# jenndrei/BayHunter

Hardware: AMD Instinct MI355X
Metric: forward-model+logL evals/sec (batched 10-layer models) (higher is better)
Workload: dtype f64

## Files before the change

bayhunter_amd/csrc/swd_fa.h:

```cpp
#pragma once

namespace fa {
constexpr double SIGN_FLOOR = 1.0e-12;

__device__ __forceinline__ void sqrt_rsqrt(double x, double &s, double &rs)
{
    const double y = __builtin_amdgcn_rsq(x);
    double g = x * y, h = 0.5 * y;
    double r = __builtin_fma(-h, g, 0.5);
    g = __builtin_fma(g, r, g);
    h = __builtin_fma(h, r, h);
    r = __builtin_fma(-h, g, 0.5);
    g = __builtin_fma(g, r, g);
    h = __builtin_fma(h, r, h);
    s = g;
    rs = h + h;
}
__device__ __forceinline__ double rcp(double x)
{
    double r = __builtin_amdgcn_rcp(x);
    r = __builtin_fma(r, __builtin_fma(-x, r, 1.0), r);
    return __builtin_fma(r, __builtin_fma(-x, r, 1.0), r);
}
__device__ __forceinline__ double rcp1(double x)
{
    const double r = __builtin_amdgcn_rcp(x);
    return __builtin_fma(r, __builtin_fma(-x, r, 1.0), r);
}

__device__ __forceinline__ void sincos(double x, double &sn, double &cs)
{
    const double n = __builtin_rint(x * 6.36619772367581382433e-01);
    double r = __builtin_fma(-n, 1.57079632673412561417e+00, x);
    r = __builtin_fma(-n, 6.07710050650619224932e-11, r);
    const double z = r * r, z2 = z * z, z4 = z2 * z2;
    const double s01 = __builtin_fma(z, 8.33333333332248946124e-03, -1.66666666666666324348e-01);
    const double s23 = __builtin_fma(z, 2.75573137070700676789e-06, -1.98412698298579493134e-04);
    const double s45 = __builtin_fma(z, 1.58969099521155010221e-10, -2.50507602534068634195e-08);
    const double ps = __builtin_fma(z4, s45, __builtin_fma(z2, s23, s01));
    const double s = __builtin_fma(r * z, ps, r);
    const double c01 = __builtin_fma(z, -1.38888888888741095749e-03, 4.16666666666666019037e-02);
    const double c23 = __builtin_fma(z, -2.75573143513906633035e-07, 2.48015872894767294178e-05);
    const double c45 = __builtin_fma(z, -1.13596475577881948265e-11, 2.08757232129817482790e-09);
    const double pc = __builtin_fma(z4, c45, __builtin_fma(z2, c23, c01));
    const double c = __builtin_fma(z2, pc, __builtin_fma(z, -0.5, 1.0));
    const int q = (int)n & 3;
    const double ss = (q & 1) ? c : s, cc = (q & 1) ? s : c;
    sn = (q & 2) ? -ss : ss;
    cs = ((q + 1) & 2) ? -cc : cc;
}
__device__ __forceinline__ double expneg(double x)
{
    const double t = -x;
    const double n = __builtin_rint(t * 1.44269504088896338700e+00);
    double r = __builtin_fma(-n, 6.93147180369123816490e-01, t);
    r = __builtin_fma(-n, 1.90821492927058770002e-10, r);
    const double r2 = r * r, r4 = r2 * r2, r8 = r4 * r4;
    const double p01 = __builtin_fma(r, 1.66666666666666666667e-01, 0.5);
    const double p23 = __builtin_fma(r, 8.33333333333333333333e-03, 4.16666666666666666667e-02);
    const double p45 = __builtin_fma(r, 1.98412698412698412698e-04, 1.38888888888888888889e-03);
    const double p67 = __builtin_fma(r, 2.75573192239858906526e-06, 2.48015873015873015873e-05);
    const double p89 = __builtin_fma(r, 2.50521083854417187751e-08, 2.75573192239858906526e-07);
    const double p03 = __builtin_fma(r2, p23, p01), p47 = __builtin_fma(r2, p67, p45);
    const double p8a = __builtin_fma(r2, 2.08767569878680989792e-09, p89);
    const double p = __builtin_fma(r8, p8a, __builtin_fma(r4, p47, p03));
    const double e = __builtin_fma(r2, p, r) + 1.0;
    return e * __longlong_as_double((long long)((unsigned long long)((long long)n + 1023ll) << 52));
}

__device__ __forceinline__ void wave(double k, double xk, double d, double &cs, double &w, double &x, double &em)
{
    const double dk = k - xk;
    const double r2 = (k + xk) * fabs(dk);
    const bool zero = !(r2 > 1.0e-290);
    double r, rr;
    sqrt_rsqrt(zero ? 1.0 : r2, r, rr);
    r = zero ? 0.0 : r;
    const double p = r * d;
    double sn;
    if (dk < 0.0) {
        sincos(fmin(p, 9.0e4), sn, cs);
        x = -(r * sn);
        em = 1.0;
    } else {
        em = expneg(fmin(p, 700.0));
        const double hf = 0.5 * (em * em);
        cs = 0.5 + hf;
        sn = 0.5 - hf;
        x = r * sn;
    }
    w = zero ? d : sn * rr;
    if (!(p < 9.0e4)) cs = __builtin_nan("");
}

__device__ __forceinline__ void layer_products(double wvno, double xka, double xkb, double dpth, LayerTerms &o)
{
    double cosp, w, x, ep, cosq, y, z, eq;
    wave(wvno, xka, dpth, cosp, w, x, ep);
    wave(wvno, xkb, dpth, cosq, y, z, eq);
    o.a0 = ep * eq;
    o.cpcq = cosp * cosq;
    o.cpy = cosp * y;
    o.cpz = cosp * z;
    o.cqw = cosq * w;
    o.cqx = cosq * x;
    o.xy = x * y;
    o.xz = x * z;
    o.wy = w * y;
    o.wz = w * z;
    o.w = w;
    o.cosp = cosp;
}

__device__ __forceinline__ void ca19(Ca19 &o, double wvno2, double gam, double gammk, double rho, double irho, const LayerTerms &v)
{
#pragma clang fp contract(fast)
    const double gamm1 = gam - 1.0;
    const double twgm1 = gam + gamm1;
    const double gmgmk = gam * gammk;
    const double gmgm1 = gam * gamm1;
    const double gm1sq = gamm1 * gamm1;
    const double rho2 = rho * rho, irho2 = irho * irho;
    const double a0pq = v.a0 - v.cpcq;
    const double ca11 = v.cpcq - 2.0 * gmgm1 * a0pq - gmgmk * v.xz - wvno2 * gm1sq * v.wy;
    const double ca12 = (wvno2 * v.cpy - v.cqx) * irho;
    const double ca13 = -(twgm1 * a0pq + gammk * v.xz + wvno2 * gamm1 * v.wy) * irho;
    const double ca14 = (v.cpz - wvno2 * v.cqw) * irho;
    const double ca15 = -(2.0 * wvno2 * a0pq + v.xz + wvno2 * wvno2 * v.wy) * irho2;
    const double ca21 = (gmgmk * v.cpz - gm1sq * v.cqw) * rho;
    const double ca23 = gammk * v.cpz - gamm1 * v.cqw;
    const double ca41 = (gm1sq * v.cpy - gmgmk * v.cqx) * rho;
    const double ca43 = gamm1 * v.cpy - gammk * v.cqx;
    const double ca51 = -(2.0 * gmgmk * gm1sq * a0pq + gmgmk * gmgmk * v.xz + gm1sq * gm1sq * v.wy) * rho2;
    const double ca53 = -(gammk * gamm1 * twgm1 * a0pq + gam * gammk * gammk * v.xz + gamm1 * gm1sq * v.wy) * rho;
    const double t = -2.0 * wvno2;
    o.c[0] = ca11; o.c[1] = ca12; o.c[2] = ca13; o.c[3] = ca14; o.c[4] = ca15;
    o.c[5] = ca21; o.c[6] = ca23; o.c[7] = -v.wz; o.c[8] = v.cpcq;
    o.c[9] = ca41; o.c[10] = -v.xy; o.c[11] = ca43;
    o.c[12] = ca51; o.c[13] = ca53;
    o.c[14] = t * ca53;
    o.c[15] = t * ca43;
    o.c[16] = v.a0 + 2.0 * (v.cpcq - ca11);
    o.c[17] = t * ca23;
    o.c[18] = t * ca13;
}

__device__ __forceinline__ void rayleigh_halfspace(double e[5], double wvno, double wvno2, double xka, double xkb, double gammk, double rho1)
{
#pragma clang fp contract(fast)
    const double ra2 = (wvno + xka) * fabs(wvno - xka), rb2 = (wvno + xkb) * fabs(wvno - xkb);
    double ra, rb, t;
    sqrt_rsqrt(ra2 > 1.0e-290 ? ra2 : 1.0, ra, t);
    sqrt_rsqrt(rb2 > 1.0e-290 ? rb2 : 1.0, rb, t);
    ra = ra2 > 1.0e-290 ? ra : 0.0;
    rb = rb2 > 1.0e-290 ? rb : 0.0;
    const double gam = gammk * wvno2;
    const double gamm1 = gam - 1.0;
    const double rarb = ra * rb;
    e[0] = rho1 * rho1 * (gamm1 * gamm1 - gam * gammk * rarb);
    e[1] = -rho1 * ra;
    e[2] = rho1 * (gamm1 - gammk * rarb);
    e[3] = rho1 * rb;
    e[4] = wvno2 - rarb;
}

__device__ __forceinline__ void normalize5(double v0, double v1, double v2, double v3, double v4, double e[5])
{
    double t1 = fmax(fmax(fmax(fabs(v0), fabs(v1)), fmax(fabs(v2), fabs(v3))), fabs(v4));
    if (t1 < 1.0e-40) t1 = 1.0;
    const double r = rcp1(t1);
    e[0] = v0 * r;
    e[1] = v1 * r;
    e[2] = v2 * r;
    e[3] = v3 * r;
    e[4] = v4 * r;
}

__device__ __forceinline__ void love_step(double &e1, double &e2, double cosq, double yx, double zx)
{
    const double e10 = __builtin_fma(e2, zx, e1 * cosq);
    const double e20 = __builtin_fma(e1, yx, e2 * cosq);
    double xnor = fmax(fabs(e10), fabs(e20));
    if (xnor < 1.0e-40) xnor = 1.0;
    const double r = rcp1(xnor);
    e1 = e10 * r;
    e2 = e20 * r;
}
__device__ __forceinline__ void love_terms(double wvno, double xkb, double dm, double &cosq, double &y, double &z, double &q)
{
    double em;
    const double dk = wvno - xkb;
    const double r2 = (wvno + xkb) * fabs(dk);
    const bool zero = !(r2 > 1.0e-290);
    double rb, rr;
    sqrt_rsqrt(zero ? 1.0 : r2, rb, rr);
    rb = zero ? 0.0 : rb;
    q = dm * rb;
    double sn;
    if (dk < 0.0) {
        sincos(fmin(q, 9.0e4), sn, cosq);
        z = -(rb * sn);
    } else {
        em = expneg(fmin(q, 700.0));
        const double hf = 0.5 * (em * em);
        cosq = 0.5 + hf;
        sn = 0.5 - hf;
        z = rb * sn;
    }
    y = zero ? dm : sn * rr;
    if (!(q < 9.0e4)) cosq = __builtin_nan("");
}

__device__ __forceinline__ void apply5(const double e[5], const double *c, double ee[5])
{
    const double ca11 = c[0], ca12 = c[1], ca13 = c[2], ca14 = c[3], ca15 = c[4];
    const double ca21 = c[5], ca23 = c[6], ca24 = c[7], ca22 = c[8];
    const double ca41 = c[9], ca42 = c[10], ca43 = c[11], ca51 = c[12], ca53 = c[13];
    const double ca31 = c[14], ca32 = c[15], ca33 = c[16], ca34 = c[17], ca35 = c[18];
    ee[0] = __builtin_fma(e[4], ca51, __builtin_fma(e[2], ca31, e[0] * ca11)) + __builtin_fma(e[3], ca41, e[1] * ca21);
    ee[1] = __builtin_fma(e[4], ca41, __builtin_fma(e[2], ca32, e[0] * ca12)) + __builtin_fma(e[3], ca42, e[1] * ca22);
    ee[2] = __builtin_fma(e[4], ca53, __builtin_fma(e[2], ca33, e[0] * ca13)) + __builtin_fma(e[3], ca43, e[1] * ca23);
    ee[3] = __builtin_fma(e[4], ca21, __builtin_fma(e[2], ca34, e[0] * ca14)) + __builtin_fma(e[3], ca22, e[1] * ca24);
    ee[4] = __builtin_fma(e[4], ca11, __builtin_fma(e[2], ca35, e[0] * ca15)) + __builtin_fma(e[3], ca12, e[1] * ca14);
}

template <class MD>
__device__ __forceinline__ double rayleigh_secular(double wvno, double omga, const MD &md, int mmax, int llw, int mtop)
{
    const double omega = omga < 1.0e-4 ? 1.0e-4 : omga;
    const double wvno2 = wvno * wvno;
    const double iom = rcp(omega);
    double e[5];
    {
        const double bh = md.Bv(mmax - 1);
        const double t = bh * iom;
        rayleigh_halfspace(e, wvno, wvno2, omega * rcp(md.A(mmax - 1)), omega * rcp(bh), 2.0 * t * t, md.R(mmax - 1));
    }
    for (int m = mtop - 2; m >= 0; --m) {
        if (m <= mmax - 2 && m >= llw - 1) {
            const double am = md.A(m), bm = md.Bv(m), rho1 = md.R(m), dpth = md.D(m);
            const double t = bm * iom;
            const double gammk = 2.0 * t * t;
            LayerTerms v;
            layer_products(wvno, omega * rcp(am), omega * rcp(bm), dpth, v);
            Ca19 c;
            ca19(c, wvno2, gammk * wvno2, gammk, rho1, rcp(rho1), v);
            double ee[5];
            apply5(e, c.c, ee);
            normalize5(ee[0], ee[1], ee[2], ee[3], ee[4], e);
        }
    }
    double result = e[0];
    if (llw != 1) {
        LayerTerms v;
        layer_products(wvno, omega * rcp(md.A(0)), wvno + 1.0, md.D(0), v);
        result = v.cosp * e[0] - md.R(0) * v.w * e[1];
    }
    return result;
}

template <class MD>
__device__ __forceinline__ double love_secular(double wvno, double omega, const MD &md, int mmax, int llw, int mtop, int *nv = nullptr)
{
    double e1, e2;
    LoveCount lc;
    {
        const double ib = rcp(md.Bv(mmax - 1));
        const double xkb = omega * ib;
        const double r2 = (wvno + xkb) * fabs(wvno - xkb);
        double rb, t_;
        sqrt_rsqrt(r2 > 1.0e-290 ? r2 : 1.0, rb, t_);
        rb = r2 > 1.0e-290 ? rb : 0.0;
        e1 = md.R(mmax - 1) * rb;
        e2 = ib * ib;
        lc.reset(wvno > xkb);
    }
    for (int m = mtop - 2; m >= 0; --m) {
        if (m <= mmax - 2 && m >= llw - 1) {
            const double beta1 = md.Bv(m), rho1 = md.R(m);
            const double ib = rcp(beta1);
            const double xkb = omega * ib;
            double cosq, y, z, q;
            love_terms(wvno, xkb, md.D(m), cosq, y, z, q);
            const double fl = (wvno < xkb) ? love_zero_floor(q) : 0.0;
            const double e2o = e2;
            love_step(e1, e2, cosq, y * (ib * ib * rcp(rho1)), z * (rho1 * beta1 * beta1));
            lc.layer(fl, e2o, e2);
        }
    }
    if (nv != nullptr) *nv = lc.packed(e1, e2);
    return e1;
}
}
```

bayhunter_amd/csrc/swd_lean.hip:

```cpp
#include "../../include/bh_engine_debug.h"
#include "bh_device.h"
#include "bh_tuning.h"
#include <algorithm>
#define BH_HD __device__ __forceinline__
#define BH_TAB static __device__ const
#include "bh_libm.h"

namespace {
#include "swd_common.h"

struct LeanModel {
    const double *p;
    int S, LS;
    __device__ __forceinline__ double D(int m) const { return p[m * S]; }
    __device__ __forceinline__ double A(int m) const { return p[LS + m * S]; }
    __device__ __forceinline__ double Bv(int m) const { return p[2 * LS + m * S]; }
    __device__ __forceinline__ double R(int m) const { return p[3 * LS + m * S]; }
    __device__ __forceinline__ double IA(int m) const { return p[4 * LS + m * S]; }
    __device__ __forceinline__ double IB(int m) const { return p[5 * LS + m * S]; }
    __device__ __forceinline__ double IR(int m) const { return p[6 * LS + m * S]; }
};

__device__ __forceinline__ double lean_rayleigh(double wvno, double omega, double iom, const LeanModel &md, int mmax, int mtop)
{
    const double wvno2 = wvno * wvno;
    double e[5];
    {
        const double t = md.Bv(mmax - 1) * iom;
        fa::rayleigh_halfspace(e, wvno, wvno2, omega * md.IA(mmax - 1), omega * md.IB(mmax - 1), 2.0 * t * t, md.R(mmax - 1));
    }
    for (int m = mtop - 2; m >= 0; --m) {
        if (m <= mmax - 2) {
            const double t = md.Bv(m) * iom;
            const double gammk = 2.0 * t * t;
            LayerTerms v;
            fa::layer_products(wvno, omega * md.IA(m), omega * md.IB(m), md.D(m), v);
            Ca19 c;
            fa::ca19(c, wvno2, gammk * wvno2, gammk, md.R(m), md.IR(m), v);
            double ee[5];
            fa::apply5(e, c.c, ee);
            if ((m & 1) == 0) {
                fa::normalize5(ee[0], ee[1], ee[2], ee[3], ee[4], e);
            } else {
#pragma unroll
                for (int i = 0; i < 5; ++i) e[i] = ee[i];
            }
        }
    }
    return e[0];
}
__device__ __forceinline__ double lean_love(double wvno, double omega, const LeanModel &md, int mmax, int mtop)
{
    double e1, e2;
    {
        const double ib = md.IB(mmax - 1);
        const double xkb = omega * ib;
        const double r2 = (wvno + xkb) * fabs(wvno - xkb);
        double rb, t_;
        fa::sqrt_rsqrt(r2 > 1.0e-290 ? r2 : 1.0, rb, t_);
        rb = r2 > 1.0e-290 ? rb : 0.0;
        e1 = md.R(mmax - 1) * rb;
        e2 = ib * ib;
    }
    for (int m = mtop - 2; m >= 0; --m) {
        if (m <= mmax - 2) {
            const double ib = md.IB(m), bm = md.Bv(m), rho1 = md.R(m);
            double cosq, y, z, q;
            fa::love_terms(wvno, omega * ib, md.D(m), cosq, y, z, q);
            fa::love_step(e1, e2, cosq, y * (ib * ib * md.IR(m)), z * (rho1 * bm * bm));
        }
    }
    return e1;
}

enum : int {
    PH_START = 0,
    PH_SCAN = 1,
    PH_REF1 = 2,
    PH_REFC = 3,
    PH_PROBE_STEP = 4,
    PH_PROBE_ACC = 5,
    PH_SPECIAL = 6,
    PH_PROBE_START = 7,
    PH_SPECIAL_B = 8,
    PH_SPECIAL_C = 9
};

__device__ __forceinline__ bool sign_neg(double x) { return __double_as_longlong(x) < 0; }
__device__ __forceinline__ void lean_wave_sync()
{
    __builtin_amdgcn_fence(__ATOMIC_RELEASE, "wavefront");
    __builtin_amdgcn_wave_barrier();
    __builtin_amdgcn_fence(__ATOMIC_ACQUIRE, "wavefront");
}

#ifndef BH_LEAN_CLUSTER_W
#define BH_LEAN_CLUSTER_W 4.0e-7
#endif
#ifndef BH_LEAN_RIDE_TOL
#define BH_LEAN_RIDE_TOL 4.0e-7
#endif
#ifndef BH_LEAN_CLUSTER_BIG
#define BH_LEAN_CLUSTER_BIG 8
#endif
#ifndef BH_LEAN_CLUSTER
#define BH_LEAN_CLUSTER 2
#endif
constexpr int LEAN_WPB = 4;

template <int J, bool CNT>
__global__ __launch_bounds__(BH_WAVE * LEAN_WPB) void swd_lean_kernel(SwdMultiArgs A, int wave_lds, int flip)
{
    if (A.started != nullptr && threadIdx.x == 0) atomicAdd(A.started, 1u);
    const int lane = threadIdx.x & (BH_WAVE - 1);
    const int wave = __builtin_amdgcn_readfirstlane((int)(threadIdx.x / BH_WAVE));
    int wid = (int)blockIdx.x * LEAN_WPB + wave, ty = (int)blockIdx.y;
    if (A.wg_n1 > 0) {
        const long long n1 = A.wg_n1, N = (long long)A.wg_n0 + n1;
        if (wid >= (int)N) return;
        const int l0 = (int)(((long long)wid * n1) / N), l1 = (int)((((long long)wid + 1) * n1) / N);
        ty = (l1 > l0) ? 1 : 0;
        wid = (l1 > l0) ? l0 : wid - l0;
        if ((flip & 256) && ty == 1) {
            if (flip & 2048) {
                const int x = (wid >> 1) & 7, q = ((wid >> 4) << 1) | (wid & 1), qr = A.wg_n1 / 8 - 1 - q;
                wid = ((qr >> 1) << 4) + 2 * x + (qr & 1);
            } else {
                wid = A.wg_n1 - 1 - wid;
            }
        }
    }
    const SwdTarget T = A.t[ty];
    constexpr int MPW = BH_WAVE / J;
    if (wid * MPW >= A.B) return;
    const int g = lane / J, r = lane & (J - 1), lbase = lane & ~(J - 1);
    const int sidx = wid * MPW + g;
    const bool valid = sidx < A.B;
    const int32_t *perm = T.perm != nullptr ? T.perm : A.perm;
    const int ib = valid ? (perm ? perm[sidx] : sidx) : 0;
    const int Lmax = A.Lmax, K = T.K, ifunc = T.iwave;
    extern __shared__ __align__(16) unsigned char smem_lean[];
    double *omg = reinterpret_cast<double *>(smem_lean + (size_t)wave * wave_lds);
    double *mdl = omg + ((K + 1) & ~1);
    const int LS = Lmax * MPW;
    constexpr double dc = (double)0.005f, onea = (double)1.5f, twopi = 2.0 * 3.141592653589793, guard_rel = 3.0e-6;
    for (int k = lane; k < K; k += BH_WAVE) omg[k] = twopi / T.periods[k];
    for (int idx = lane; idx < LS; idx += BH_WAVE) {
        const int l = idx / MPW, mg = idx - l * MPW;
        const int sb = wid * MPW + mg;
        const int b = sb < A.B ? (perm ? perm[sb] : sb) : 0;
        float fd = 0.f, fa_ = 1.f, fb = 1.f, fr = 1.f;
        if (sb < A.B && l < A.nlay[b]) {
            const ptrdiff_t o = (ptrdiff_t)b * T.sb + (ptrdiff_t)l * T.sl;
            fd = (float)T.h[o];
            fa_ = (float)T.vp[o];
            fb = (float)T.vs[o];
            fr = (float)T.rho[o];
        }
        mdl[idx] = (double)fd;
        mdl[LS + idx] = (double)fa_;
        mdl[2 * LS + idx] = (double)fb;
        mdl[3 * LS + idx] = (double)fr;
        mdl[4 * LS + idx] = fa::rcp((double)fa_);
        mdl[5 * LS + idx] = fa::rcp((double)fb);
        mdl[6 * LS + idx] = fa::rcp((double)fr);
    }
    int mmax = valid ? A.nlay[ib] : 2;
    mmax = mmax < 1 ? 1 : (mmax > Lmax ? Lmax : mmax);
    int mtop = mmax;
    for (int off = 32; off > 0; off >>= 1) mtop = max(mtop, __shfl_xor(mtop, off));
    mtop = __builtin_amdgcn_readfirstlane(mtop);
    lean_wave_sync();
    LeanModel md;
    md.p = mdl + g;
    md.S = MPW;
    md.LS = LS;

    float betmx = -1.e20f, betmn = 1.e20f;
    int jmn = 0, jsol = 1;
    bool sane = true;
    for (int i = 0; i < mmax; ++i) {
        const float bi = (float)md.Bv(i), ai = (float)md.A(i), di = (float)md.D(i), ri = (float)md.R(i);
        sane = sane && (ai > 0.0f) && (ai <= 100.0f) && (bi >= 0.0f) && (bi <= 100.0f) && (ri > 0.0f) && (ri < 1.0e6f) &&
               (i == mmax - 1 || (di >= 0.0f && di < 1.0e7f));
        if (bi > 0.01f && bi < betmn) {
            betmn = bi;
            jmn = i;
            jsol = 1;
        } else if (bi <= 0.01f && ai < betmn) {
            betmn = ai;
            jmn = i;
            jsol = 0;
        }
        if (bi > betmx) betmx = bi;
    }
    float cc1 = (jsol == 0) ? betmn : gtsolh_f32((float)md.A(jmn), (float)md.Bv(jmn));
    cc1 = 0.95f * cc1;
    cc1 = 0.90f * cc1;
    const double cm = (double)cc1, betmxd = (double)betmx;
    const double vh0 = md.Bv(mmax - 1), vh1 = (ifunc == 2) ? md.A(mmax - 1) : betmxd, vsafe = fmin(vh0, vh1);
    auto special_in_cell = [&](double lo_, double hi_) -> double {
        double sp = 0.0;
        int n = 0;
        if (lo_ < betmxd && betmxd < hi_) sp = betmxd, ++n;
        if (vh0 != betmxd && lo_ < vh0 && vh0 < hi_) sp = vh0, ++n;
        if (vh1 != betmxd && vh1 != vh0 && lo_ < vh1 && vh1 < hi_) sp = vh1, ++n;
        return n > 1 ? -1.0 : sp;
    };
    double *vel = T.vel + (size_t)ib * T.ldv;
    const bool writer = valid && r == 0;
    bool active = valid && K > 0 && sane, guard = false;
#define LEAN_GUARD(n) do { guard = true; if (CNT) greason = (n); } while (0)
    int greason = 0;
    int errflag = 0;
    if (valid && !sane) {
        errflag = 1;
        if (writer)
            for (int i = 0; i < K; ++i) vel[i] = 0.0;
    }
    if (active && md.Bv(0) <= 0.0) {
        LEAN_GUARD(1);
        active = false;
    }
    int k = 0, ph = PH_START, idir = +1, ifirst = 1, nref = 0;
    double c1 = cm, clow = cm, del1 = 0.0, ck = 0.0, omega = 1.0, iom = 1.0;
    bool s1stneg = false;
    double cp = 0.0, delp = 0.0;
    bool havep = false;
    double lo = 0.0, hi = 0.0, flo = 0.0, fhi = 0.0, p3 = 0.0, fp3 = 0.0, c3 = 0.0, wprev = 0.0;
    bool have3 = false;
    double cell_lo = 0.0, cell_hi = 0.0, pb = 0.0, delb = 0.0;
    bool pp_neg = false;
    int sp_nb = 0;
    bool flo_neg = false, chk = false;
    unsigned evals = 0;
    if (active) {
        omega = omg[0];
        iom = fa::rcp(omega);
    }
    constexpr unsigned long long maskJ = (J >= 64) ? ~0ull : ((1ull << J) - 1ull);
    constexpr int NC = (J >= 32) ? BH_LEAN_CLUSTER_BIG : ((J >= 8) ? BH_LEAN_CLUSTER : J / 2), NR = J - NC;
    constexpr bool can_spec = J >= 4;
    constexpr unsigned long long maskC = (1ull << NC) - 1ull, maskR = (1ull << NR) - 1ull;
    const double invJ1 = 1.0 / (double)(J + 1);
    unsigned nrounds = 0;
    long long t_eval = 0;
    const long long t_start = ((CNT && A.neval != nullptr)) ? clock64() : 0;
    while (__ballot(active) != 0ull) {
        ++nrounds;
        double cev = c1, cprev = c1;
        double om_l = omega, iom_l = iom;
        bool pt = false;
        bool spec = false;
        double xc = 0.0;
        if (ph <= PH_SCAN) {
            const bool start = ph == PH_START;
            if (!start) {
                if (idir > 0) {
                    if (c1 + dc <= clow) c1 = clow;
                } else if (c1 - dc <= clow) {
                    idir = +1;
                    c1 = clow;
                    havep = false;
                }
            }
            const double base = (start && c1 + dc <= clow) ? clow : c1;
            const int n = start ? r : r + 1;
            const double step = (idir > 0 || start) ? dc : -dc;
            cprev = __builtin_fma((double)(n - 1), step, base);
            cev = (n == 0) ? c1 : __builtin_fma((double)n, step, base);
        } else if (ph == PH_REF1) {
            cev = __builtin_fma(hi - lo, (double)(r + 1) * invJ1, lo);
            pt = cev > lo && cev < hi;
        } else if (ph == PH_REFC) {
            double x = 0.0;
            bool ok = false;
            if (have3) {
                const double d12 = flo - fhi, d1p = flo - fp3, d2p = fhi - fp3;
                const double den = d12 * d1p * d2p;
                if (den != 0.0) {
                    const double id = fa::rcp(den);
                    x = (lo * fhi * fp3 * d2p - hi * flo * fp3 * d1p + p3 * flo * fhi * d12) * id;
                    ok = x > lo && x < hi;
                }
            }
            if (!ok) {
                x = lo - flo * (hi - lo) * fa::rcp(fhi - flo);
                if (!(x > lo && x < hi)) x = 0.5 * (lo + hi);
            }
            spec = can_spec && k + 1 < K;
            xc = x;
            const int nc = spec ? NC : J;
            if (r < nc) {
                const int h = nc / 2;
                const double w = ((spec && NC == 2) ? BH_LEAN_CLUSTER_W : 1.0e-7) * fabs(x);
                cev = (r < h) ? x - __builtin_ldexp(w, 2 * (h - 1 - r)) : x + __builtin_ldexp(w, 2 * (r - h));
                pt = cev > lo && cev < hi;
            } else {
                const int s_ = r - NC;
                const double c1n = x - onea * dc;
                const double basen = (c1n + dc <= cm) ? cm : c1n;
                cprev = __builtin_fma((double)(s_ - 1), dc, basen);
                cev = (s_ == 0) ? c1n : __builtin_fma((double)s_, dc, basen);
                om_l = omg[k + 1];
                iom_l = fa::rcp(om_l);
            }
        } else if (J >= 32 && (ph == PH_SPECIAL || ph == PH_SPECIAL_B)) {
            const double sp = special_in_cell(cell_lo, cell_hi);
            const double g = guard_rel * sp;
            const bool up = ph == PH_SPECIAL_B;
            const float lg = log2f((float)(((up ? cell_hi - sp : sp - cell_lo)) / g)) * (1.0f / (float)(J - 1));
            const double dist = g * (double)exp2f(lg * (float)(r - 1));
            cev = (r == 0) ? (up ? sp + g : sp - g) : ((r == 1) ? sp + g : (up ? sp + dist : sp - dist));
        } else if (J >= 32 && ph == PH_SPECIAL_C) {
            const double sp = special_in_cell(cell_lo, cell_hi);
            const double dist = (1.0e-8 * sp) * (double)exp2f((8.2288187f / (float)(J / 2)) * (float)(r >> 1));
            cev = (r & 1) ? sp + dist : sp - dist;
        } else if (ph == PH_PROBE_START) {
            cev = (r == 0) ? c1 - guard_rel * c1 : ((r == 1) ? c1 + guard_rel * c1 : c1);
        } else if (ph == PH_PROBE_STEP) {
            const double l_ = fmin(c1, pb), h_ = fmax(c1, pb);
            cev = (r == 0) ? l_ + guard_rel * h_ : h_ - guard_rel * h_;
        } else {
            cev = (r == 0) ? cell_hi + guard_rel * fabs(c3) : cell_lo - guard_rel * fabs(c3);
        }
        if (!active || !(cev > 0.0)) cev = 1.0;
        const long long te0 = ((CNT && A.neval != nullptr)) ? clock64() : 0;
        const double wvno = om_l * fa::rcp(cev);
        const double del = (ifunc == 2) ? lean_rayleigh(wvno, om_l, iom_l, md, mmax, mtop) : lean_love(wvno, om_l, md, mmax, mtop);
        if ((CNT && A.neval != nullptr)) t_eval += clock64() - te0;

        const bool dneg = sign_neg(del);
        const unsigned long long mneg = (__ballot(dneg) >> lbase) & maskJ;
        const unsigned long long m_small = (__ballot(!(fabs(del) >= fa::SIGN_FLOOR)) >> lbase) & maskJ;
        const unsigned long long m_pt = (__ballot(pt) >> lbase) & maskJ;
        const bool inB = ph == PH_REFC && spec && r >= NC;
        int ev = 0;
        if (ph <= PH_SCAN || inB) {
            const bool first = ph == PH_START || inB;
            const int rr = inB ? r - NC : r;
            if (!(first && rr == 0)) {
                const bool down = !first && idir < 0;
                const double a_ = fmin(cprev, cev), b_ = fmax(cprev, cev);
                const bool refneg = inB ? ((mneg >> NC) & 1ull) != 0ull : (first ? (mneg & 1ull) != 0ull : sign_neg(del1));
                const double floor_ = inB ? cm : clow;
                if (down && cev <= floor_) ev = 1;
                else if (dneg != refneg) ev = 2;
                else if (b_ >= vsafe && ((a_ <= vh0 && vh0 <= b_) || (a_ <= vh1 && vh1 <= b_))) ev = 3;
                else if (cev < cm || cev >= betmxd + dc) ev = 4;
            }
        } else if (ph <= PH_REFC) {
            ev = (pt && dneg != sign_neg(flo)) ? 2 : 0;
        }
        const unsigned long long m_ev = (__ballot(ev != 0) >> lbase) & maskJ;
        const int nA = (ph == PH_REFC && spec) ? NC : J;
        const unsigned long long m_evA = (ph == PH_REFC && spec) ? (m_ev & maskC) : m_ev;
        const int eA = m_evA ? (int)__builtin_ctzll(m_evA) : nA;
        const int r0 = m_pt ? (int)__builtin_ctzll(m_pt) : 0, r1 = m_pt ? 63 - (int)__builtin_clzll(m_pt) : -1;
        const int i3 = (eA < nA) ? ((eA + 1 <= r1) ? eA + 1 : eA - 2) : r1 - 1;
        const double dA_e = __shfl(del, lbase + (eA < nA ? eA : nA - 1)), dA_1 = __shfl(del, lbase + (eA > 0 ? eA - 1 : 0));
        const double d_3 = __shfl(del, lbase + (i3 >= 0 && i3 < J ? i3 : 0)), d_r1 = __shfl(del, lbase + (r1 >= 0 ? r1 : 0));

        int todo = 0;
        bool scan_now = false;
        int w0 = 0;
        bool sc_first = false;
        bool special_now = false;
        if (J >= 32 && __ballot(active && ph == PH_SPECIAL_C) != 0ull) {
            if (active && ph == PH_SPECIAL_C) {
                special_now = true;
                evals += (unsigned)J;
                if (m_small != 0ull || mneg != (pp_neg ? maskJ : 0ull)) {
                    LEAN_GUARD(6);
                } else if (sp_nb != 0) {
                    todo = 2;
                } else {
                    have3 = false;
                    nref = 0;
                    wprev = hi - lo;
                    ph = PH_REFC;
                }
            }
        }
        if (J >= 32 && __ballot(active && (ph == PH_SPECIAL || ph == PH_SPECIAL_B)) != 0ull) {
            const bool up = ph == PH_SPECIAL_B;
            const bool s_near = up ? pp_neg : (mneg & 1ull) != 0ull, s_end = up ? !flo_neg : flo_neg;
            const unsigned long long inner = (J > 2) ? ((mneg >> 2) & ((1ull << (J - 2)) - 1ull)) : 0ull;
            const unsigned long long seq = (s_near ? 1ull : 0ull) | (inner << 1) | ((s_end ? 1ull : 0ull) << (J - 1));
            const unsigned long long ch = (seq ^ (seq >> 1)) & ((1ull << (J - 1)) - 1ull);
            const int nch = __builtin_popcountll(ch);
            const int te = ch ? (int)__builtin_ctzll(ch) : 0;
            const int e_near = (te == 0) ? (up ? 1 : 0) : te + 1, e_far = (te + 1 == J - 1) ? -1 : te + 2;
            const double d_near = __shfl(del, lbase + e_near), d_far = __shfl(del, lbase + (e_far < 0 ? 0 : e_far));
            const double c_near = __shfl(cev, lbase + e_near), c_far = __shfl(cev, lbase + (e_far < 0 ? 0 : e_far));
            if (active && (ph == PH_SPECIAL || ph == PH_SPECIAL_B)) {
                special_now = true;
                evals += (unsigned)J;
                const bool is_betmx = special_in_cell(cell_lo, cell_hi) == betmxd;
                if (m_small != 0ull || nch > 1) {
                    LEAN_GUARD(6);
                } else if (!up) {
                    pp_neg = (mneg & 2ull) != 0ull;
                    if (pp_neg != ((mneg & 1ull) != 0ull)) LEAN_GUARD(6);
                    sp_nb = nch;
                    if (nch == 1) {
                        hi = c_near;
                        fhi = d_near;
                        if (e_far >= 0) {
                            lo = c_far;
                            flo = d_far;
                        }
                    }
                    ph = PH_SPECIAL_B;
                } else {
                    if (sp_nb + nch != 1) {
                        if (is_betmx && sp_nb == 0 && nch > 0) todo = 2;
                        else LEAN_GUARD(6);
                    } else {
                        sp_nb = (nch == 1 && is_betmx) ? 1 : 0;
                        if (nch == 1) {
                            lo = c_near;
                            flo = d_near;
                            if (e_far >= 0) {
                                hi = c_far;
                                fhi = d_far;
                            }
                        }
                        ph = PH_SPECIAL_C;
                    }
                }
            }
        }
        if (active) {
            scan_now = ph <= PH_SCAN;
            sc_first = ph == PH_START;
            bool probed = false;
            if (special_now) {
            } else if (ph == PH_PROBE_STEP) {
                evals += 2;
                const bool n1 = sign_neg(del1);
                if ((m_small & 3ull) || ((mneg & 1ull) != 0ull) != n1 || ((mneg & 2ull) != 0ull) != n1) {
                    LEAN_GUARD(4);
                } else {
                    cp = c1;
                    delp = del1;
                    havep = true;
                    c1 = pb;
                    del1 = delb;
                    ph = PH_SCAN;
                    if (c1 < cm || c1 >= betmxd + dc) todo = 2;
                }
            } else if (ph == PH_REF1 || ph == PH_REFC) {
                const double olo = lo, ohi = hi, oflo = flo, ofhi = fhi;
                const int nc = nA, h = nc / 2;
                const double w = ((nA == 2) ? BH_LEAN_CLUSTER_W : 1.0e-7) * fabs(xc);
                const bool sect = ph == PH_REF1;
                auto ctrial = [&](int i) -> double {
                    return sect ? __builtin_fma(ohi - olo, (double)(i + 1) * invJ1, olo)
                                : ((i < h) ? xc - __builtin_ldexp(w, 2 * (h - 1 - i)) : xc + __builtin_ldexp(w, 2 * (i - h)));
                };
                evals += (unsigned)__builtin_popcountll(m_pt);
                ++nref;
                if (sect && m_pt != 0ull) {
                    const int np = r1 - r0 + 1;
                    const unsigned long long sg = (mneg >> r0) & ((np >= 64) ? ~0ull : ((1ull << np) - 1ull));
                    const int inner = __builtin_popcountll((sg ^ (sg >> 1)) & ((np >= 65) ? ~0ull : ((1ull << (np - 1)) - 1ull)));
                    const int ends = ((((sg & 1ull) != 0ull) != sign_neg(oflo)) ? 1 : 0) + (((((sg >> (np - 1)) & 1ull) != 0ull) != sign_neg(ofhi)) ? 1 : 0);
                    if (inner + ends > 1) LEAN_GUARD(6);
                }
                if (m_pt != 0ull) {
                    if (eA < nA) {
                        hi = ctrial(eA);
                        fhi = dA_e;
                        if (eA - 1 >= r0) {
                            lo = ctrial(eA - 1);
                            flo = dA_1;
                        }
                    } else {
                        lo = ctrial(r1);
                        flo = d_r1;
                    }
                    if (i3 >= r0 && i3 <= r1) {
                        p3 = ctrial(i3);
                        fp3 = d_3;
                        have3 = true;
                    } else if (hi != ohi) {
                        p3 = ohi;
                        fp3 = ofhi;
                        have3 = true;
                    } else if (lo != olo) {
                        p3 = olo;
                        fp3 = oflo;
                        have3 = true;
                    }
                }
                const bool poor = ph == PH_REFC && (hi - lo > 0.25 * wprev || (nref == 1 && !(eA > 0 && eA < nA)));
                if (poor && nref == 1) {
                    lo = olo;
                    hi = ohi;
                    flo = oflo;
                    fhi = ofhi;
                }
                ph = poor ? PH_REF1 : PH_REFC;
                wprev = hi - lo;
                if (hi - lo <= 1.3e-6 * fabs(hi) || nref >= 16 || m_pt == 0ull) {
                    c3 = lo - flo * (hi - lo) * fa::rcp(fhi - flo);
                    if (have3) {
                        const double d12 = flo - fhi, d1p = flo - fp3, d2p = fhi - fp3;
                        const double den = d12 * d1p * d2p;
                        const double xq = (lo * fhi * fp3 * d2p - hi * flo * fp3 * d1p + p3 * flo * fhi * d12) * fa::rcp(den);
                        if (den != 0.0 && xq >= lo && xq <= hi) c3 = xq;
                    }
                    if (!(c3 >= lo && c3 <= hi)) c3 = 0.5 * (lo + hi);
                    todo = 3;
                }
            } else if (ph == PH_PROBE_START) {
                evals += 3;
                const bool nA = (mneg & 1ull) != 0ull, nB = (mneg & 2ull) != 0ull, n2 = (mneg & 4ull) != 0ull;
                if ((m_small & 7ull) || (nA != nB && nA != s1stneg) || (nA == nB && n2 != nA)) LEAN_GUARD(2);
                ph = PH_START;
                chk = true;
            } else if (ph == PH_PROBE_ACC) {
                evals += 2;
                if ((m_small & 3ull) || ((mneg & 1ull) != 0ull) == flo_neg || ((mneg & 2ull) != 0ull) != flo_neg) LEAN_GUARD(5);
                todo = 4;
                probed = true;
            }
            if (todo == 3) {
                const double m2 = 2.0 * dc;
                todo = 4;
                if (fabs(c3 - vh0) < m2 || fabs(c3 - vh1) < m2 || fabs(c3 - betmxd) < m2) {
                    const double eps = guard_rel * fabs(c3);
                    if (cell_hi - c3 < eps || c3 - cell_lo < eps || fabs(c3 - betmxd) < eps) {
                        LEAN_GUARD(7);
                    } else {
                        ph = PH_PROBE_ACC;
                        todo = 0;
                    }
                }
            }
            if (guard) {
                active = false;
                todo = 0;
            }
            if (todo == 4) {
                if (c3 > betmxd) {
                    todo = 2;
                } else {
                    ck = c3;
                    if (writer) vel[k] = (double)(float)ck;
                    k = k + 1;
                    if (k >= K) {
                        active = false;
                    } else {
                        omega = omg[k];
                        iom = fa::rcp(omega);
                        ifirst = 0;
                        c1 = ck - onea * dc;
                        clow = cm;
                        ph = PH_START;
                        if (!probed && spec && fabs(c3 - xc) <= BH_LEAN_RIDE_TOL * fabs(c3)) {
                            c1 = xc - onea * dc;
                            scan_now = true;
                            sc_first = true;
                            w0 = NC;
                        }
                    }
                }
            }
            if (todo == 2) {
                errflag = 1;
                if (writer)
                    for (int i = k; i < K; ++i) vel[i] = 0.0;
                active = false;
            }
        }
        const int wn = (w0 != 0) ? NR : J;
        const unsigned long long m_evS = (w0 != 0) ? ((m_ev >> NC) & maskR) : m_ev;
        const int e = m_evS ? (int)__builtin_ctzll(m_evS) : wn;
        const int wb = lbase + w0;
        const int ev_e = __shfl(ev, wb + (e < wn ? e : wn - 1));
        const double d_e = __shfl(del, wb + (e < wn ? e : wn - 1)), d_em = __shfl(del, wb + (e > 0 ? e - 1 : 0)),
                     d_em2 = __shfl(del, wb + (e > 1 ? e - 2 : 0)), d_first = __shfl(del, wb), d_second = __shfl(del, wb + 1);
        if (active && scan_now) {
            const bool start = sc_first;
            const unsigned long long msm = (w0 != 0) ? ((m_small >> NC) & maskR) : m_small;
            const double base = (start && c1 + dc <= clow) ? clow : c1;
            const double step = (start || idir > 0) ? dc : -dc;
            const double c1s = c1;
            auto cgrid = [&](int t) -> double { return (start && t == 0) ? c1s : __builtin_fma((double)(start ? t : t + 1), step, base); };
            int off = 0, todo2 = 0;
            bool consume = true;
            const bool look_closer = start && !chk && ifirst != 1 && !(msm & 1ull) && !(flip & 4096) && fabs(d_first) < 1.0e-2 * fabs(d_second - d_first);
            if (look_closer) {
                ph = PH_PROBE_START;
                consume = false;
            } else if (start) {
                chk = false;
                ++evals;
                if (msm & 1ull) LEAN_GUARD(2);
                del1 = d_first;
                havep = false;
                if (ifirst == 1) s1stneg = sign_neg(d_first);
                idir = (ifirst != 1 && s1stneg != sign_neg(d_first)) ? -1 : +1;
                off = 1;
                if (idir > 0) {
                    if (c1 + dc <= clow) {
                        c1 = clow;
                        havep = false;
                    }
                } else {
                    consume = false;
                }
                ph = PH_SCAN;
            }
            if (consume) {
                const int last = (e < wn) ? ((ev_e == 1) ? e - 1 : e) : wn - 1;
                if (last >= off) {
                    evals += (unsigned)(last - off + 1);
                    const unsigned long long used = ((last >= 63) ? ~0ull : ((1ull << (last + 1)) - 1ull)) & ~((1ull << off) - 1ull);
                    if (msm & used) LEAN_GUARD(3);
                }
                const int ns = e - off;
                if (ns >= 2) {
                    cp = cgrid(e - 2);
                    delp = d_em2;
                    havep = true;
                } else if (ns == 1) {
                    cp = c1;
                    delp = del1;
                    havep = true;
                }
                if (ns >= 1) {
                    c1 = cgrid(e - 1);
                    del1 = d_em;
                }
                if (e < wn) {
                    if (ev_e == 1) {
                        idir = +1;
                        c1 = clow;
                        havep = false;
                    } else if (ev_e == 2) {
                        pb = cgrid(e);
                        delb = d_e;
                        todo2 = 1;
                    } else if (ev_e == 3) {
                        pb = cgrid(e);
                        delb = d_e;
                        ph = PH_PROBE_STEP;
                    } else {
                        todo2 = 2;
                    }
                }
            }
            if (todo2 == 1) {
                cell_lo = fmin(c1, pb);
                cell_hi = fmax(c1, pb);
                flo = (c1 < pb) ? del1 : delb;
                fhi = (c1 < pb) ? delb : del1;
                flo_neg = sign_neg(flo);
                lo = cell_lo;
                hi = cell_hi;
                p3 = cp;
                fp3 = delp;
                have3 = havep;
                nref = 0;
                wprev = hi - lo;
                ph = have3 ? PH_REFC : PH_REF1;
                {
                    const double sp = special_in_cell(cell_lo, cell_hi);
                    if (sp != 0.0) {
                        ph = PH_SPECIAL;
                        if (J < 32 || !(sp > 0.0 && sp - guard_rel * sp > cell_lo && sp + guard_rel * sp < cell_hi)) LEAN_GUARD(6);
                    } else if (cell_lo > vsafe) {
                        have3 = false;
                        ph = PH_REF1;
                    }
                }
            }
            if (guard) active = false;
            if (todo2 == 2 && active) {
                errflag = 1;
                if (writer)
                    for (int i = k; i < K; ++i) vel[i] = 0.0;
                active = false;
            }
        }
    }
    if (writer) {
        T.err[ib] = errflag;
        if (guard && T.gcount != nullptr) {
            T.glist[atomicAdd(T.gcount, 1)] = ib;
            atomicAdd(T.gcount + 2 * BH_MAX_TARGETS, 1);
        }
    }
    if ((CNT && A.neval != nullptr)) {
        unsigned long long tot = writer ? evals : 0u, lps = tot * (unsigned long long)(valid ? mmax - 1 : 0);
        for (int off = 32; off > 0; off >>= 1) {
            tot += __shfl_xor(tot, off);
            lps += __shfl_xor(lps, off);
        }
        if (lane == 0) {
            atomicAdd(A.neval, tot);
            atomicAdd(A.neval + (ifunc == 2 ? 8 : 9), tot);
            atomicAdd(A.neval + (ifunc == 2 ? 10 : 11), lps);
            const int o = (ifunc == 2) ? 1 : 4;
            atomicAdd(A.neval + o, (unsigned long long)nrounds);
            atomicAdd(A.neval + o + 1, (unsigned long long)(clock64() - t_start));
            atomicMax(A.neval + o + 2, (unsigned long long)nrounds);
            atomicAdd(A.neval + 7, 1ull);
            atomicAdd(A.neval + (ifunc == 2 ? 12 : 13), (unsigned long long)t_eval);
        }
        if (writer && guard && greason >= 1 && greason <= 7)
            atomicAdd(A.neval + (greason <= 4 ? 14 : 15), 1ull << (16 * ((greason - 1) & 3)));
    }
}
}

static size_t lean_wave_lds(int J, int Lmax, int Kmax)
{
    return ((((size_t)((Kmax + 1) & ~1) + (size_t)7 * Lmax * (BH_WAVE / J)) * sizeof(double)) + 15) & ~(size_t)15;
}
size_t bh_swd_lean_lds_bytes(int J, int Lmax, int Kmax) { return LEAN_WPB * lean_wave_lds(J, Lmax, Kmax); }

int bh_swd_lean_trials(int B, int nt)
{
    const long pairs = (long)B * nt;
    return pairs <= 1024 ? 64 : (pairs <= 5120 ? 32 : (pairs <= 10240 ? 16 : (pairs <= 28672 ? 8 : 4)));
}

int bh_launch_swd_lean(const SwdMultiArgs &a0, hipStream_t stream, SwdLaunchInfo *info)
{
    SwdMultiArgs a = a0;
    int kmax = 0, jmin = BH_WAVE;
    long wmax = 1, wsum = 0, nw[BH_MAX_TARGETS] = {0};
    for (int t = 0; t < a.ntargets; ++t) {
        const int J = a.t[t].look;
        if (J < 4 || J > BH_WAVE || (J & (J - 1)) != 0 || a.t[t].igr != 0 || a.t[t].mode > 1) return -1;
        kmax = a.t[t].K > kmax ? a.t[t].K : kmax;
        jmin = J < jmin ? J : jmin;
        const int mpw = BH_WAVE / J;
        nw[t] = (a.B + mpw - 1) / mpw;
        wmax = nw[t] > wmax ? nw[t] : wmax;
        wsum += nw[t];
    }
    const size_t wave_lds = lean_wave_lds(jmin, a.Lmax, kmax);
    const size_t lds = LEAN_WPB * wave_lds;
    if (lds > 64 * 1024) return -1;
    dim3 grid((unsigned)((wmax + LEAN_WPB - 1) / LEAN_WPB), (unsigned)a.ntargets);
    a.wg_n0 = a.wg_n1 = 0;
    if (a.ntargets == 2) {
        a.wg_n0 = (int)nw[0];
        a.wg_n1 = (int)nw[1];
        grid = dim3((unsigned)((wsum + LEAN_WPB - 1) / LEAN_WPB), 1);
    }
    const dim3 block(BH_WAVE * LEAN_WPB);
    if (info != nullptr) {
        info->workgroups = grid.x * grid.y;
        info->waves = wsum;
        info->lds = lds;
        info->fast_arith = 1;
        info->restarts_in_place = 0;
    }
    int flip = bh_tuning().swd_lean_flip;
    if (a.ntargets == 2 && nw[0] == nw[1] && nw[1] % 16 == 0) flip |= 2048;
    const int J = a.t[0].look;
    for (int t = 1; t < a.ntargets; ++t)
        if (a.t[t].look != J) return -1;
    const bool cnt = a.neval != nullptr;
#define LEAN_LAUNCH(JJ)                                                                                                             \
    do {                                                                                                                            \
        if (cnt) hipLaunchKernelGGL((swd_lean_kernel<JJ, true>), grid, block, lds, stream, a, (int)wave_lds, flip);                 \
        else hipLaunchKernelGGL((swd_lean_kernel<JJ, false>), grid, block, lds, stream, a, (int)wave_lds, flip);                    \
    } while (0)
    switch (J) {
    case 4: LEAN_LAUNCH(4); break;
    case 8: LEAN_LAUNCH(8); break;
    case 16: LEAN_LAUNCH(16); break;
    case 32: LEAN_LAUNCH(32); break;
    default: LEAN_LAUNCH(64); break;
    }
#undef LEAN_LAUNCH
    return 0;
}
```

Measured before the change: 6.103 million.

## Fold per-layer density scaling into precomputed interface ratios for Rayleigh and Love

```diff
diff --git a/bayhunter_amd/csrc/swd_fa.h b/bayhunter_amd/csrc/swd_fa.h
--- a/bayhunter_amd/csrc/swd_fa.h
+++ b/bayhunter_amd/csrc/swd_fa.h
@@ -65,7 +65,7 @@
     const double p8a = __builtin_fma(r2, 2.08767569878680989792e-09, p89);
     const double p = __builtin_fma(r8, p8a, __builtin_fma(r4, p47, p03));
     const double e = __builtin_fma(r2, p, r) + 1.0;
-    return e * __longlong_as_double((long long)((unsigned long long)((long long)n + 1023ll) << 52));
+    return e * __hiloint2double(((int)n + 1023) << 20, 0);
 }
 
 __device__ __forceinline__ void wave(double k, double xk, double d, double &cs, double &w, double &x, double &em)
@@ -145,6 +145,38 @@
     o.c[18] = t * ca13;
 }
 
+__device__ __forceinline__ void ca19u(Ca19 &o, double wvno2, double gam, double gammk, const LayerTerms &v)
+{
+#pragma clang fp contract(fast)
+    const double gamm1 = gam - 1.0;
+    const double twgm1 = gam + gamm1;
+    const double gmgmk = gam * gammk;
+    const double gmgm1 = gam * gamm1;
+    const double gm1sq = gamm1 * gamm1;
+    const double a0pq = v.a0 - v.cpcq;
+    const double ca11 = v.cpcq - 2.0 * gmgm1 * a0pq - gmgmk * v.xz - wvno2 * gm1sq * v.wy;
+    const double ca12 = wvno2 * v.cpy - v.cqx;
+    const double ca13 = -(twgm1 * a0pq + gammk * v.xz + wvno2 * gamm1 * v.wy);
+    const double ca14 = v.cpz - wvno2 * v.cqw;
+    const double ca15 = -(2.0 * wvno2 * a0pq + v.xz + wvno2 * wvno2 * v.wy);
+    const double ca21 = gmgmk * v.cpz - gm1sq * v.cqw;
+    const double ca23 = gammk * v.cpz - gamm1 * v.cqw;
+    const double ca41 = gm1sq * v.cpy - gmgmk * v.cqx;
+    const double ca43 = gamm1 * v.cpy - gammk * v.cqx;
+    const double ca51 = -(2.0 * gmgmk * gm1sq * a0pq + gmgmk * gmgmk * v.xz + gm1sq * gm1sq * v.wy);
+    const double ca53 = -(gammk * gamm1 * twgm1 * a0pq + gam * gammk * gammk * v.xz + gamm1 * gm1sq * v.wy);
+    const double t = -2.0 * wvno2;
+    o.c[0] = ca11; o.c[1] = ca12; o.c[2] = ca13; o.c[3] = ca14; o.c[4] = ca15;
+    o.c[5] = ca21; o.c[6] = ca23; o.c[7] = -v.wz; o.c[8] = v.cpcq;
+    o.c[9] = ca41; o.c[10] = -v.xy; o.c[11] = ca43;
+    o.c[12] = ca51; o.c[13] = ca53;
+    o.c[14] = t * ca53;
+    o.c[15] = t * ca43;
+    o.c[16] = v.a0 + 2.0 * (v.cpcq - ca11);
+    o.c[17] = t * ca23;
+    o.c[18] = t * ca13;
+}
+
 __device__ __forceinline__ void rayleigh_halfspace(double e[5], double wvno, double wvno2, double xka, double xkb, double gammk, double rho1)
 {
 #pragma clang fp contract(fast)
@@ -185,6 +217,16 @@
     const double r = rcp1(xnor);
     e1 = e10 * r;
     e2 = e20 * r;
+}
+__device__ __forceinline__ void love_step_scaled(double &e1, double &h, double cosq, double y, double z, double x)
+{
+    const double e10 = __builtin_fma(h, z, e1 * cosq);
+    const double e20 = __builtin_fma(e1, y, h * cosq) * x;
+    double xnor = fmax(fabs(e10), fabs(e20));
+    if (xnor < 1.0e-40) xnor = 1.0;
+    const double r = rcp1(xnor);
+    e1 = e10 * r;
+    h = e20 * r;
 }
 __device__ __forceinline__ void love_terms(double wvno, double xkb, double dm, double &cosq, double &y, double &z, double &q)
 {
diff --git a/bayhunter_amd/csrc/swd_lean.hip b/bayhunter_amd/csrc/swd_lean.hip
--- a/bayhunter_amd/csrc/swd_lean.hip
+++ b/bayhunter_amd/csrc/swd_lean.hip
@@ -18,7 +18,7 @@
     __device__ __forceinline__ double R(int m) const { return p[3 * LS + m * S]; }
     __device__ __forceinline__ double IA(int m) const { return p[4 * LS + m * S]; }
     __device__ __forceinline__ double IB(int m) const { return p[5 * LS + m * S]; }
-    __device__ __forceinline__ double IR(int m) const { return p[6 * LS + m * S]; }
+    __device__ __forceinline__ double X(int m) const { return p[6 * LS + m * S]; }
 };
 
 __device__ __forceinline__ double lean_rayleigh(double wvno, double omega, double iom, const LeanModel &md, int mmax, int mtop)
@@ -29,6 +29,13 @@
         const double t = md.Bv(mmax - 1) * iom;
         fa::rayleigh_halfspace(e, wvno, wvno2, omega * md.IA(mmax - 1), omega * md.IB(mmax - 1), 2.0 * t * t, md.R(mmax - 1));
     }
+    if (mmax >= 2) {
+        const double rt = md.R(mmax - 2);
+        e[1] *= rt;
+        e[2] *= rt;
+        e[3] *= rt;
+        e[4] *= rt * rt;
+    }
     for (int m = mtop - 2; m >= 0; --m) {
         if (m <= mmax - 2) {
             const double t = md.Bv(m) * iom;
@@ -36,15 +43,11 @@
             LayerTerms v;
             fa::layer_products(wvno, omega * md.IA(m), omega * md.IB(m), md.D(m), v);
             Ca19 c;
-            fa::ca19(c, wvno2, gammk * wvno2, gammk, md.R(m), md.IR(m), v);
+            fa::ca19u(c, wvno2, gammk * wvno2, gammk, v);
             double ee[5];
             fa::apply5(e, c.c, ee);
-            if ((m & 1) == 0) {
-                fa::normalize5(ee[0], ee[1], ee[2], ee[3], ee[4], e);
-            } else {
-#pragma unroll
-                for (int i = 0; i < 5; ++i) e[i] = ee[i];
-            }
+            const double x = md.X(m), x2 = x * x;
+            fa::normalize5(ee[0], ee[1] * x, ee[2] * x, ee[3] * x, ee[4] * x2, e);
         }
     }
     return e[0];
@@ -61,13 +64,16 @@
         rb = r2 > 1.0e-290 ? rb : 0.0;
         e1 = md.R(mmax - 1) * rb;
         e2 = ib * ib;
+        if (mmax >= 2) {
+            const double bt = md.Bv(mmax - 2);
+            e2 *= md.R(mmax - 2) * bt * bt;
+        }
     }
     for (int m = mtop - 2; m >= 0; --m) {
         if (m <= mmax - 2) {
-            const double ib = md.IB(m), bm = md.Bv(m), rho1 = md.R(m);
             double cosq, y, z, q;
-            fa::love_terms(wvno, omega * ib, md.D(m), cosq, y, z, q);
-            fa::love_step(e1, e2, cosq, y * (ib * ib * md.IR(m)), z * (rho1 * bm * bm));
+            fa::love_terms(wvno, omega * md.IB(m), md.D(m), cosq, y, z, q);
+            fa::love_step_scaled(e1, e2, cosq, y, z, md.X(m));
         }
     }
     return e1;
@@ -163,7 +169,13 @@
         mdl[3 * LS + idx] = (double)fr;
         mdl[4 * LS + idx] = fa::rcp((double)fa_);
         mdl[5 * LS + idx] = fa::rcp((double)fb);
-        mdl[6 * LS + idx] = fa::rcp((double)fr);
+    }
+    lean_wave_sync();
+    for (int idx = lane; idx < LS; idx += BH_WAVE) {
+        const double mu = (ifunc == 2) ? mdl[3 * LS + idx] : mdl[3 * LS + idx] * mdl[2 * LS + idx] * mdl[2 * LS + idx];
+        const double mu_up = (idx < MPW) ? 1.0
+                           : ((ifunc == 2) ? mdl[3 * LS + idx - MPW] : mdl[3 * LS + idx - MPW] * mdl[2 * LS + idx - MPW] * mdl[2 * LS + idx - MPW]);
+        mdl[6 * LS + idx] = mu_up * fa::rcp(mu);
     }
     int mmax = valid ? A.nlay[ib] : 2;
     mmax = mmax < 1 ? 1 : (mmax > Lmax ? Lmax : mmax);
```

Result: no change. 6.141 million, median of 6 (+0.6%).
